# rafaelsoStanford/State_Policy_DiffusionModel

Hardware: AMD Instinct MI355X
Metric: denoise-steps/sec (B=4096, horizon=32) (higher is better)
Workload: dtype f32 (split-fp16 MFMA operands, fp32 accumulate)

## Files before the change

state_policy_diffusionmodel_amd/csrc/conv_gemm.hip:

```cpp
#include <algorithm>
#include <cstdlib>

#include "device_utils.h"

namespace spdm {

typedef float f32x16 __attribute__((ext_vector_type(16)));
typedef float f32x4 __attribute__((ext_vector_type(4)));
typedef float f32x2 __attribute__((ext_vector_type(2)));
typedef unsigned u32x2 __attribute__((ext_vector_type(2)));
typedef _Float16 f16x8 __attribute__((ext_vector_type(8)));
typedef _Float16 f16x4 __attribute__((ext_vector_type(4)));

constexpr float SPLIT_ACT_SCALE = 16.0f;
constexpr float SPLIT_DESCALE = 1.0f / 2048.0f;

typedef _Float16 f16x2 __attribute__((ext_vector_type(2)));
__device__ __forceinline__ f32x2 split_pair(float a, float b) {
    unsigned h, l;
    split_pair_f16(a * SPLIT_ACT_SCALE, b * SPLIT_ACT_SCALE, h, l);
    return f32x2{__builtin_bit_cast(float, h), __builtin_bit_cast(float, l)};
}

constexpr int CK = 32;
// ... 563 lines not shown
                v += bias4;
                if (epi == EPI_BIAS_GELU) {
                    v.x = gelu_erf(v.x); v.y = gelu_erf(v.y); v.z = gelu_erf(v.z); v.w = gelu_erf(v.w);
                }
                if (epi == EPI_BIAS_RESID)
                    v += *reinterpret_cast<const f32x4*>(a.resid + (size_t)row * a.resid_ld + n0 + c4o * 4);
                *reinterpret_cast<f32x4*>(dstp + (size_t)row * dst_ld + n0 + c4o * 4) = v;
                if (a.row_stats != nullptr) {
                    float s1 = (v.x + v.y) + (v.z + v.w);
                    float s2 = (v.x * v.x + v.y * v.y) + (v.z * v.z + v.w * v.w);
#pragma unroll
                    for (int o2 = TPR >> 1; o2 > 0; o2 >>= 1) {
                        s1 += __shfl_xor(s1, o2, 64);
                        s2 += __shfl_xor(s2, o2, 64);
                    }
                    if (c4o == 0) {
                        double* rs = a.row_stats + ((size_t)row * n_ntiles + ntile) * 2;
                        rs[0] = (double)s1;
                        rs[1] = (double)s2;
                    }
                }
            }
        }
    }
    SPDM_STAMP()
#ifdef SPDM_DIAG
    if (stamping) a.stamps[(tid >> 8) * 128 + 127] = (unsigned long long)nstamp;
#endif
#undef SPDM_STAMP
#undef SPDM_ROW
}

int spdm_tune(int idx, int dflt) {
    constexpr int NT = 26;
    static int val[NT];
    static bool have[NT], init = false;
    if (!init) {
        for (int i = 0; i < NT; ++i) {
            char name[20];
            snprintf(name, sizeof(name), "SPDM_TUNE%d", i);
            const char* e = getenv(name);
            have[i] = e != nullptr;
            val[i] = e ? atoi(e) : 0;
        }
        init = true;
    }
    return (idx >= 0 && idx < NT && have[idx]) ? val[idx] : dflt;
}

GemmGeom gemm_geometry(int M, int N, int K, int HW, int W, int taps, int split, unsigned sw, bool stats_epi) {
    GemmGeom g;
    g.skinny = 0;
    g.reg = 0;
    if (stats_epi && conv_reg_geometry(M, N, K, HW, W, taps, split, sw)) {
        g.reg = 1;
        g.m_tile = 64; g.n_tile = 64; g.n_tiles = 1; g.ksplit = 1;
        g.st_m_tile = 64; g.st_n_tiles = 1;
        g.slots = stats_slots(HW, 64, 1);
        return g;
    }
    if (stats_epi && taps != 1 && conv_skinny_geometry(M, N, K, HW, W, taps, split, sw, &g.m_tile, &g.n_tile)) {
        g.skinny = 1;
        g.ksplit = 1;
        g.n_tiles = N / g.n_tile;
        g.st_m_tile = g.m_tile;
        g.st_n_tiles = g.n_tiles;
        g.slots = stats_slots(HW, g.st_m_tile, g.st_n_tiles);
// ... 80 lines not shown
    return conv_wide_takes_upcat(b, g);
}

bool gemm_takes_two_sources(const GemmArgs& a0) {
    if (a0.skip == nullptr || !a0.split || a0.wgt_frag == nullptr || (a0.sw & SW_NO_FUSED_SRC) || a0.epi != EPI_STATS) return false;
    GemmArgs a = a0;
    const GemmGeom g = gemm_geometry(a);
    if (g.skinny || g.reg || g.m_tile == 512) return false;
    a.ksplit = g.ksplit;
    return conv_wide_supported(a, g);
}

static bool uses_w2(const GemmArgs& a, const GemmGeom& g) {
    return a.split && g.m_tile == 256 && a.taps == 9 && a.W == 2 && a.HW % 2 == 0 && !(a.sw & SW_NO_W2);
}
static bool uses_wp4(const GemmArgs& a0, const GemmGeom& g) {
    if (!(a0.split && a0.taps == 9 && a0.W == 4 && g.n_tile == 128 && (g.m_tile == 128 || g.m_tile == 256) && a0.HW % 16 == 0 &&
          a0.K % 64 == 0 && !(a0.sw & SW_NO_WP4)) || g.skinny) return false;
    GemmArgs a = a0;
    a.ksplit = g.ksplit;
    return conv_wide_supported(a, g);
}
static bool uses_wp8(const GemmArgs& a0, const GemmGeom& g) {
    if (!(a0.split && a0.taps == 9 && a0.W == 8 && g.n_tile == 128 && g.m_tile == 256 && a0.HW % 32 == 0 && a0.K % 64 == 0 &&
          !(a0.sw & SW_NO_WP8)) || g.skinny) return false;
    GemmArgs a = a0;
    a.ksplit = g.ksplit;
    return conv_wide_supported(a, g);
}
double gemm_flops(const GemmArgs& a0) {
    GemmArgs a = a0;
    const GemmGeom g = gemm_geometry(a.geom_M > 0 ? a.geom_M : a.M, a.N, a.K, a.HW, a.W, a.taps, a.split, a.sw, a.epi == EPI_STATS);
    if (a.pro == PRO_UPCAT && !g.skinny && gemm_takes_fused_source(a0)) a.pro = a.skip_stats.p != nullptr ? PRO_GN : PRO_NONE;
    const double taps = uses_w2(a, g) ? 6.0 : uses_wp4(a, g) ? 7.5 : uses_wp8(a, g) ? 8.25 : (double)a.taps;
    return 2.0 * (double)a.M * (double)a.N * (double)a.K * taps;
}

template <bool HALO, int PREC, int WM, int WN, int MT, int NT, int TPI, bool W2 = false, bool DEEP = false>
static hipError_t launch_cfg(const GemmArgs& a, const GemmGeom& g, hipStream_t s) {
    constexpr int M_T = WM * MT * 32, N_T = WN * NT * 32, NTHR = WM * WN * 64;
    constexpr int NBA = (TPI == 1 || DEEP) ? 2 : 1;
    const int halo = HALO ? a.W + 1 : 0;
    const int QA = M_T + 2 * halo;
    const int NSP = (QA + 4) & ~3;
#ifdef SPDM_WDMA
    constexpr bool WDMA = (NTHR == 512) && (PREC == PREC_SPLIT);
#else
    constexpr bool WDMA = false;
#endif
    constexpr int WROW = WDMA ? 32 : LDK;
    size_t lds = (size_t)(NBA * (QA + 1) * LDK + 2 * TPI * N_T * WROW + 2 * NSP) * sizeof(float);
    lds = std::max(lds, (size_t)(M_T * WN * 2 + M_T * N_T) * sizeof(float));
    if (lds > 160 * 1024 || g.m_tile != M_T || g.n_tile != N_T) return hipErrorInvalidValue;
    auto kern = conv_gemm_kernel<HALO, PREC, WM, WN, MT, NT, TPI, W2, DEEP>;
    if (hipError_t e = allow_full_lds(reinterpret_cast<const void*>(kern)); e != hipSuccess) return e;
    const int n_mtiles = (a.M + M_T - 1) / M_T;
    const int grid = n_mtiles * g.n_tiles * std::max(a.ksplit, 1);
    if (a.route) *a.route = GemmRoute{ROUTE_GEMM, W2 ? VAR_W2 : VAR_PLAIN, M_T, N_T};
    hipLaunchKernelGGL(kern, dim3(grid), dim3(NTHR), lds, s, a, g.slots);
    return hipGetLastError();
}

static hipError_t launch_gemm_kernel(const GemmArgs& a, const GemmGeom& g, hipStream_t s);

static int g_wide_upcat_launches = 0;
int gemm_wide_upcat_launches() { return g_wide_upcat_launches; }

// ... 80 lines not shown
```

state_policy_diffusionmodel_amd/csrc/conv_wide.hip:

```cpp
#include <algorithm>
#include <cstdlib>

#include "device_utils.h"
#include "resample.h"

namespace spdm {

typedef float f32x16 __attribute__((ext_vector_type(16)));
typedef float f32x4 __attribute__((ext_vector_type(4)));
typedef float f32x2 __attribute__((ext_vector_type(2)));
typedef _Float16 f16x8 __attribute__((ext_vector_type(8)));
typedef _Float16 f16x2 __attribute__((ext_vector_type(2)));

namespace {

constexpr float ACT_SCALE = 16.0f;
constexpr float DESCALE = 1.0f / 2048.0f;
constexpr int CK = 32;
#ifndef WIDE_LDS_PERM
#define WIDE_LDS_PERM 1
#endif
template <bool W2, bool PIPE = false, bool WP = false> struct WidePitch { static constexpr int value = (W2 || PIPE || WP || !WIDE_LDS_PERM) ? 36 : 40; };
constexpr bool wp_active(int t, int rt) { return !((t % 3 == 0 && (rt & 3) == 0) || (t % 3 == 2 && (rt & 3) == 3)); }
constexpr int wp_first(int t) { return (t % 3 == 0) ? 1 : 0; }
// ... 12 lines not shown
#ifndef WIDE_STAGE_GROUP
#define WIDE_STAGE_GROUP 1
#endif
#ifndef WIDE_DB
#define WIDE_DB 0
#endif
#ifndef WIDE_EARLY
#define WIDE_EARLY 0
#endif
#ifndef WIDE_NH
#define WIDE_NH 2
#endif

__device__ __forceinline__ f32x2 split2(float a, float b) {
    unsigned h, l;
    split_pair_f16(a * ACT_SCALE, b * ACT_SCALE, h, l);
    return f32x2{__builtin_bit_cast(float, h), __builtin_bit_cast(float, l)};
}

template <int NT, int PRO, bool W2, int RT, int WN, bool PIPE, bool TWO = false, int WP = 0, bool G2 = false, int WH = 0, bool UP = false>
#ifndef WIDE_MINB
#define WIDE_MINB 2
#endif
__global__ __launch_bounds__(256, WIDE_MINB) void conv3x3_wide_kernel(const GemmArgs a, const int epi_slots, const int NS) {
    constexpr int WM = 4 / WN;
    constexpr int CT = 2 * NT;
    constexpr int RW = RT * 16;
    constexpr int NTHR = 256;
    constexpr int RP = NTHR / 8;
    constexpr int M_T = WM * RW, N_T = WN * NT * 32;
    constexpr bool WHOLE = (WH != 0);
    constexpr bool ONE = (WH == 2);
    constexpr int APASS = WHOLE ? M_T / RP : (M_T + 18 + RP - 1) / RP;
    constexpr int FAR = (W2 || WP) ? 4 : 3;
    constexpr int FBR = (NT == 2) ? 2 : 3;
    constexpr int PH = 3 * NT;
    constexpr int BB = (APASS <= 9) ? 7 : (APASS <= 10) ? 6 : 5;
    static_assert(APASS * BB <= 64, "sample-index packing");
    static_assert(!W2 || NT == 2, "the width-2 variant exists for 128-wide tiles");
    static_assert(RT == 8 || (RT == 4 && NT == 2 && !W2), "64-row waves only in the tap-pair loop");
    static_assert(WN == 2 || (WN == 1 && RT == 4), "the 4 x 1 wave arrangement uses 64-row waves");
    static_assert(!TWO || (!PIPE && PRO != PRO_GN_GELU), "two-source input: first conv of a block, plain hand-over");
    static_assert(WP == 0 || WP == 4 || WP == 8, "row permutation for width-4 or width-8 maps");
    static_assert(!WP || (NT == 2 && WN == 2 && !W2 && !PIPE), "row permutation: 128-wide tiles");
    static_assert((16 + 4 * (WP == 8 ? 7 : 6)) % 4 == 0, "A ring phase");
    static_assert(WP != 8 || RT == 8, "width-8 maps: one 128-row block per wave");
    constexpr bool WP8 = (WP == 8);
    constexpr int NI8 = (M_T + 18 + 6) / 8 + 1;
    static_assert(!G2 || (NT == 2 && RT == 4 && !W2 && !PIPE && !WP && !WIDE_DB), "two chunks per hand-over: the plain tap loop, 64 rows per wave");
    static_assert(!WHOLE || (!G2 && !WIDE_DB && !WIDE_EARLY), "whole-sample staging: not in the hand-over experiments");
    static_assert(!UP || (TWO && WHOLE && RT == 8 && NT == 2 && WN == 2 && (W2 || WP)), "upsample in the loader: whole-sample two-source 256-row tiles");
    constexpr int UW = WP8 ? 8 : WP ? 4 : 2;
    constexpr int UPASS = M_T / 4 / RP;
    constexpr int RAWP = 36;
    extern __shared__ __attribute__((aligned(16))) float smem[];

    const int tid = threadIdx.x, lane = tid & 63;
    const int wave = __builtin_amdgcn_readfirstlane(tid >> 6);
    const int wm = wave / WN, wn = wave % WN, l16 = lane & 15, kg = lane >> 4;
    const int HW = a.HW, W = a.W, H = a.H, M = a.M, K = a.K, N = a.N;
    const int halo = WHOLE ? 0 : W + 1;
    const int QA = M_T + 2 * halo;
    const int QZ = WP8 ? 8 * NI8 + 2 : QA + 2;

    const int n_ntiles = N / N_T;
    const int nblk = gridDim.x, bid = blockIdx.x;
    const int q8 = nblk >> 3, r8 = nblk & 7, xcd = bid & 7, idx = bid >> 3;
    const int logical = (xcd < r8 ? xcd * (q8 + 1) : r8 * (q8 + 1) + (xcd - r8) * q8) + idx;
    const int ksp = a.ksplit > 1 ? a.ksplit : 1;
    const int tiles_mn = nblk / ksp;
    const int ks = logical / tiles_mn, tl = logical - ks * tiles_mn;
    const int mtile = tl / n_ntiles, ntile = tl - mtile * n_ntiles;
    const int m0 = mtile * M_T, n0 = ntile * N_T;
    const int kc0 = 2 * (int)((long long)ks * (K / (2 * CK)) / ksp), kc1 = (ksp > 1) ? 2 * (int)((long long)(ks + 1) * (K / (2 * CK)) / ksp) : K / CK;

    static_assert(!PIPE || (NT == 2 && !W2), "the pipelined hand-over exists in the tap loop of 128-wide tiles");
    constexpr int LDK = WidePitch<W2, PIPE, (WP != 0) || G2>::value;
// ... 242 lines not shown
        acc[rt_][(ct0_)] = __builtin_amdgcn_mfma_f32_16x16x32_f16(fa[fas_][0], fb[fbs_][0][0], acc[rt_][(ct0_)], 0, 0, 0);         \
        acc[rt_][(ct0_) + 1] = __builtin_amdgcn_mfma_f32_16x16x32_f16(fa[fas_][0], fb[fbs_][1][0], acc[rt_][(ct0_) + 1], 0, 0, 0); \
        acc[rt_][(ct0_)] = __builtin_amdgcn_mfma_f32_16x16x32_f16(fa[fas_][0], fb[fbs_][0][1], acc[rt_][(ct0_)], 0, 0, 0);         \
        acc[rt_][(ct0_) + 1] = __builtin_amdgcn_mfma_f32_16x16x32_f16(fa[fas_][0], fb[fbs_][1][1], acc[rt_][(ct0_) + 1], 0, 0, 0); \
        acc[rt_][(ct0_)] = __builtin_amdgcn_mfma_f32_16x16x32_f16(fa[fas_][1], fb[fbs_][0][0], acc[rt_][(ct0_)], 0, 0, 0);         \
        acc[rt_][(ct0_) + 1] = __builtin_amdgcn_mfma_f32_16x16x32_f16(fa[fas_][1], fb[fbs_][1][0], acc[rt_][(ct0_) + 1], 0, 0, 0); \
    }

    const int nrows = (kc1 - kc0) * 3;
    f16x8 fa[FAR][2], fb[FBR][2][2];
#define WIDE_SHIFT(kr_, dwi_) (WP8 ? (((dwi_) - 1) * NI8 + ((kr_) - 1)) * LDK : (((kr_) - 1) * W + ((dwi_) - 1)) * LDK)

    if constexpr (!W2 && NT == 2 && !(WP && RT == 8)) {
        f16x8 fbt[2][4][2], fat[2][2];
#define TAP_LOAD_B(slot_, chunk_, tap_)                                                              \
        if (!dbg_no_wload) {                                                                         \
            const float* p_ = wfl + (size_t)((tap_) * nchunks + (chunk_)) * wtap;                    \
            _Pragma("unroll") for (int c_ = 0; c_ < 4; ++c_) {                                      \
                fbt[slot_][c_][0] = *reinterpret_cast<const f16x8*>(p_ + c_ * 512);                  \
                fbt[slot_][c_][1] = *reinterpret_cast<const f16x8*>(p_ + c_ * 512 + 256);            \
            }                                                                                        \
        }
#define TAP_LOAD_FA(slot_, tap_, shift_, rt_)                                                        \
        {                                                                                            \
            const unsigned mb_ = (am[(rt_) / 3] >> (9 * ((rt_) % 3) + (tap_))) & 1u;                 \
            const int o_ = mb_ ? aoff0 + WIDE_ROWOFF(rt_) * LDK + (shift_) : zoff;                   \
            fat[slot_][0] = *reinterpret_cast<const f16x8*>(Abuf + o_);                              \
            fat[slot_][1] = *reinterpret_cast<const f16x8*>(Abuf + o_ + 16);                         \
        }
        const int TAPS = a.taps;
        const bool t3 = (TAPS == 3);
#define TAP_SHIFT(tap_) (t3 ? ((tap_) - 1) * W * LDK : (((tap_) / 3 - 1) * W + ((tap_) - ((tap_) / 3) * 3 - 1)) * LDK)
#define TAP_BIT(tap_) (t3 ? 3 * (tap_) + 1 : (tap_))
        if constexpr (WP) {
#define WP_SHIFT(t_) ((((t_) / 3 - 1) * W + ((t_) % 3 - 1)) * LDK)
            TAP_LOAD_B(0, kc0, 0)
            WIDE_LOAD_A(kc0)
            WIDE_STAGE_A()
            __syncthreads();
            WIDE_STAMP(2)
            int aoff_w = aoff0;
#define WP_LOAD_FA(slot_, tap_, shift_, rt_)                                                         \
            {                                                                                        \
                const unsigned mb_ = (am[(rt_) / 3] >> (9 * ((rt_) % 3) + (tap_))) & 1u;             \
                const int o_ = mb_ ? aoff_w + WIDE_ROWOFF(rt_) * LDK + (shift_) : zoff;              \
                fat[slot_][0] = *reinterpret_cast<const f16x8*>(Abuf + o_);                          \
                fat[slot_][1] = *reinterpret_cast<const f16x8*>(Abuf + o_ + 16);                     \
            }
            WP_LOAD_FA(0, 0, WP_SHIFT(0), wp_first(0))
            for (int chunk = kc0; chunk < kc1; ++chunk) {
                const int cn1 = min(chunk + 1, kc1 - 1);
                asm volatile("" : "+v"(aoff_w));
#pragma unroll
                for (int i = 0; i < (RT + 2) / 3; ++i) asm volatile("" : "+v"(am[i]));
#pragma unroll
                for (int t = 0; t < 9; ++t) {
                    if (t < 8) { TAP_LOAD_B((t + 1) & 1, chunk, t + 1) } else { TAP_LOAD_B(1, cn1, 0) }
#pragma unroll
                    for (int rt = 0; rt < RT; ++rt) {
                        {
                            if (wp_active(t, rt)) {
                                const int g = wp_order(t, rt, RT);
                                const int nx = wp_next(t, rt, RT);
                                if (nx >= 0) { WP_LOAD_FA((g + 1) & 1, t, WP_SHIFT(t), nx) }
                                else if (t < 8) { WP_LOAD_FA((g + 1) & 1, t + 1, WP_SHIFT(t + 1), wp_first(t + 1)) }
                                __builtin_amdgcn_sched_barrier(0);
                                if (!dbg_no_mfma) {
// ... 58 lines not shown
                    const int bi_ = WHOLE ? ((pass_) * RP + srow_p) >> lhw : (int)((abidx >> (BB * (pass_))) & ((1ull << BB) - 1)); \
                    const float rs_ = srstd[bi_], mu_ = smean[bi_];                                  \
                    v_.x = (v_.x - mu_) * (rs_ * g4r.x) + b4r.x;                                     \
                    v_.y = (v_.y - mu_) * (rs_ * g4r.y) + b4r.y;                                     \
                    v_.z = (v_.z - mu_) * (rs_ * g4r.z) + b4r.z;                                     \
                    v_.w = (v_.w - mu_) * (rs_ * g4r.w) + b4r.w;                                     \
                }                                                                                    \
                if (pro) {                                                                           \
                    if (pro_gelu) {                                                                  \
                        v_.x = gelu_erf(v_.x); v_.y = gelu_erf(v_.y);                                \
                        v_.z = gelu_erf(v_.z); v_.w = gelu_erf(v_.w);                                \
                    }                                                                                \
                }                                                                                    \
                if (!WHOLE && !((avalid >> (pass_)) & 1u)) v_ = f32x4{0.f, 0.f, 0.f, 0.f};              \
                const f32x2 p0_ = split2(v_.x, v_.y), p1_ = split2(v_.z, v_.w);                      \
                float* row_ = Awr + (WHOLE ? (pass_) * RP + srow_p : min((pass_) * RP + srow_p, QA + 1)) * LDK; \
                *reinterpret_cast<f32x2*>(row_ + c4 * 2) = f32x2{p0_.x, p1_.x};                      \
                *reinterpret_cast<f32x2*>(row_ + 16 + c4 * 2) = f32x2{p0_.y, p1_.y};                 \
            }
#define PIPE_SHIFT(t_) ((((t_) / 3 - 1) * W + ((t_) % 3 - 1)) * LDK)
            TAP_LOAD_B(0, kc0, 0)
            WIDE_LOAD_A(kc0)
            WIDE_STAGE_A()
            __syncthreads();
            { float* t_ = Abuf; Abuf = Awr; Awr = t_; }
            {
                const int c1 = min(kc0 + 1, kc1 - 1);
                PIPE_LOAD(0, c1, 0)
                PIPE_LOAD(1, c1, 1)
                PIPE_LOAD(2, c1, 2)
                PIPE_GB(c1)
            }
            WIDE_STAMP(2)
            PIPE_LOAD_FA(0, 0, PIPE_SHIFT(0), 0)
            for (int chunk = kc0; chunk < kc1; ++chunk) {
                const int cn1 = min(chunk + 1, kc1 - 1), cn2 = min(chunk + 2, kc1 - 1);
                PIPE_OPAQUE()
#pragma unroll
                for (int t = 0; t < 9; ++t) {
                    if (t < 8) { TAP_LOAD_B((t + 1) & 1, chunk, t + 1) } else { TAP_LOAD_B(1, cn1, 0) }
                    if (t < APASS) { PIPE_STAGE(t % 3, t) }
                    if (t + 3 < APASS) { PIPE_LOAD(t % 3, cn1, t + 3) }
                    else if (t >= 6) { PIPE_LOAD(t - 6, cn2, t - 6) }
                    if (t == 8) { PIPE_GB(cn2) }
#pragma unroll
                    for (int rt = 0; rt < RT; ++rt) {
                        if (rt + 1 < RT) { PIPE_LOAD_FA((rt + 1) & 1, t, PIPE_SHIFT(t), rt + 1) }
                        else if (t < 8) { PIPE_LOAD_FA(0, t + 1, PIPE_SHIFT(t + 1), 0) }
                        __builtin_amdgcn_sched_barrier(0);
#pragma unroll
                        for (int c = 0; c < 4; ++c)
                            acc[rt][c] = __builtin_amdgcn_mfma_f32_16x16x32_f16(fat[rt & 1][0], fbt[t & 1][c][0], acc[rt][c], 0, 0, 0);
#pragma unroll
                        for (int c = 0; c < 4; ++c)
                            acc[rt][c] = __builtin_amdgcn_mfma_f32_16x16x32_f16(fat[rt & 1][0], fbt[t & 1][c][1], acc[rt][c], 0, 0, 0);
#pragma unroll
                        for (int c = 0; c < 4; ++c)
                            acc[rt][c] = __builtin_amdgcn_mfma_f32_16x16x32_f16(fat[rt & 1][1], fbt[t & 1][c][0], acc[rt][c], 0, 0, 0);
                        __builtin_amdgcn_sched_barrier(0);
                    }
                }
                __syncthreads();
                { float* t_ = Abuf; Abuf = Awr; Awr = t_; }
#pragma unroll
                for (int c = 0; c < 4; ++c) { fbt[0][c][0] = fbt[1][c][0]; fbt[0][c][1] = fbt[1][c][1]; }
                PIPE_LOAD_FA(0, 0, PIPE_SHIFT(0), 0)
            }
#undef PIPE_OPAQUE
#undef PIPE_LOAD_FA
#undef PIPE_LOAD
#undef PIPE_GB
#undef PIPE_STAGE
#undef PIPE_SHIFT
        } else if constexpr (G2) {
        const int ntaps = (kc1 - kc0) * TAPS;
        f32x4 areg2[APASS];
        f32x4 g4r2 = {1.f, 1.f, 1.f, 1.f}, b4r2 = {0.f, 0.f, 0.f, 0.f};
        bool ident2 = false;
        const float* Acur = Abuf;
#define G2_LOAD_FA(slot_, tap_, shift_, rt_)                                                         \
        {                                                                                            \
            const unsigned mb_ = (am[(rt_) / 3] >> (9 * ((rt_) % 3) + (tap_))) & 1u;                 \
            const int o_ = mb_ ? aoff0 + WIDE_ROWOFF(rt_) * LDK + (shift_) : zoff;                   \
            fat[slot_][0] = *reinterpret_cast<const f16x8*>(Acur + o_);                              \
            fat[slot_][1] = *reinterpret_cast<const f16x8*>(Acur + o_ + 16);                         \
        }
        TAP_LOAD_B(0, kc0, 0)
        WIDE_LOAD_A_(kc0, areg, g4r, b4r, ident)
        WIDE_LOAD_A_(min(kc0 + 1, kc1 - 1), areg2, g4r2, b4r2, ident2)
        WIDE_STAGE_A_(areg, g4r, b4r, ident, Abuf)
        WIDE_STAGE_A_(areg2, g4r2, b4r2, ident2, Abuf + QZ * LDK)
        __syncthreads();
        WIDE_STAMP(2)
        G2_LOAD_FA(0, TAP_BIT(0), TAP_SHIFT(0), 0)
        int chunk = kc0, tap = 0;
        for (int tt = 0; tt < ntaps; tt += 2) {
#pragma unroll
            for (int half = 0; half < 2; ++half) {
                int ntap = tap + 1, nchunk = chunk;
// ... 66 lines not shown
                    __builtin_amdgcn_sched_barrier(0);
                    if (!dbg_no_mfma) {
#pragma unroll
                        for (int c = 0; c < 4; ++c)
                            acc[rt][c] = __builtin_amdgcn_mfma_f32_16x16x32_f16(fat[rt & 1][0], fbt[half][c][0], acc[rt][c], 0, 0, 0);
#pragma unroll
                        for (int c = 0; c < 4; ++c)
                            acc[rt][c] = __builtin_amdgcn_mfma_f32_16x16x32_f16(fat[rt & 1][0], fbt[half][c][1], acc[rt][c], 0, 0, 0);
#pragma unroll
                        for (int c = 0; c < 4; ++c)
                            acc[rt][c] = __builtin_amdgcn_mfma_f32_16x16x32_f16(fat[rt & 1][1], fbt[half][c][0], acc[rt][c], 0, 0, 0);
                    }
                    __builtin_amdgcn_sched_barrier(0);
                }
                if (next_A && !dbg_no_aload) {
                    if (!(DB && WIDE_EARLY)) { WIDE_LOAD_A(nchunk) }
                    if (!DB) __syncthreads();
                    WIDE_STAGE_A()
                    __syncthreads();
                    if (DB) { float* t_ = Abuf; Abuf = Awr; Awr = t_; }
                    TAP_LOAD_FA(0, TAP_BIT(0), TAP_SHIFT(0), 0)
                } else if (next_A) {
                    TAP_LOAD_FA(0, TAP_BIT(0), TAP_SHIFT(0), 0)
                }
                tap = ntap;
                chunk = nchunk;
            }
        }
        }
#undef TAP_LOAD_B
#undef TAP_LOAD_FA
#undef TAP_SHIFT
#undef TAP_BIT
    } else if constexpr (WP) {
#define WP_PLUS(i_) (WP8 ? (i_) : (i_) + (i_) / 3)
#define WP_MINUS(i_) (WP8 ? (i_) + 1 : (i_) + (i_) / 3 + 1)
        constexpr int WS = WP8 ? 7 : 6;
        constexpr int Q1 = 16 + 2 * WS, Q2 = 16 + 4 * WS;
        WIDE_LOAD_B(0, kc0, 1, 0)
        WIDE_LOAD_A(kc0)
        WIDE_STAGE_A()
        __syncthreads();
        WIDE_STAMP(2)
        WIDE_LOAD_FA(0, 1, WIDE_SHIFT(0, 1), 0)
        WIDE_LOAD_FA(1, 1, WIDE_SHIFT(0, 1), 1)
        int chunk = kc0, kr = 0;
        for (int r = 0; r < nrows; ++r) {
            int nkr = kr + 1, nchunk = chunk;
            if (nkr == 3) { nkr = 0; nchunk = chunk + 1; }
            const bool have_next = (r + 1 < nrows);
            const bool next_A = have_next && (nkr == 0);
            const int bkr = have_next ? nkr : kr, bchunk = have_next ? nchunk : chunk;
#pragma unroll
            for (int cp = 0; cp < 2; ++cp) {
                if (cp == 0) { WIDE_LOAD_B(1, chunk, kr * 3 + 1, 1) } else { WIDE_LOAD_B(0, chunk, kr * 3 + 2, 0) }
#pragma unroll
                for (int rt = 0; rt < RT; ++rt) {
                    const int q = cp * 8 + rt;
                    if (q + 2 < 16) { WIDE_LOAD_FA((q + 2) % FAR, kr * 3 + 1, WIDE_SHIFT(kr, 1), (q + 2) % 8) }
                    else { WIDE_LOAD_FA((q + 2) % FAR, kr * 3 + 2, WIDE_SHIFT(kr, 2), WP_PLUS(q + 2 - 16)) }
                    __builtin_amdgcn_sched_barrier(0);
                    WIDE_STEP(q % FAR, cp, rt, cp * 2)
                    __builtin_amdgcn_sched_barrier(0);
                }
            }
#pragma unroll
// ... 336 lines not shown
            a.skip_ld < a.K - a.up_C || a.src_ld < a.up_C) return false;
    }
    if (a.ksplit > 1 && a.K % 64 != 0) return false;
    if ((g.m_tile + 2 * (a.W + 1) - 1) / a.HW + 2 > 128) return false;
    if (g.m_tile == 128)
        return g.n_tile == 128 && (a.taps == 9 || (a.taps == 3 && a.W == 1)) && a.K % 64 == 0 && !(a.sw & SW_NO_WIDE128);
    if (g.m_tile != 256) return false;
    if (a.taps == 3) return false;
    if (a.taps != 9 || !(g.n_tile == 128 || g.n_tile == 64)) return false;
    if (wide_w2(a)) return g.n_tile == 128 && (a.HW & 7) == 0;
    if (g.n_tile == 128 && a.K % 64 != 0) return false;
    return true;
}

static GemmArgs upcat_as_two(const GemmArgs& a0) {
    GemmArgs a = a0;
    a.pro = a0.skip_stats.p != nullptr ? PRO_GN : PRO_NONE;
    return a;
}
bool conv_wide_takes_upcat(const GemmArgs& a, const GemmGeom& g) {
    if (a.pro != PRO_UPCAT || a.M <= 0 || a.skip == nullptr || a.src == nullptr || g.skinny || g.reg || g.ksplit > 1 || a.ksplit > 1) return false;
    if (g.m_tile != 256 || g.n_tile != 128 || a.taps != 9 || (a.H & 1) || a.HW != a.H * a.W || a.HW < 16 || (a.HW & (a.HW - 1)) != 0) return false;
    if ((a.sw & (SW_NO_WHOLE_TILES | SW_NO_FUSED_SRC)) || 256 % a.HW != 0 || a.M % 256 != 0 || a.K % 64 != 0) return false;
    const int level = a.W == 8 ? 0 : a.W == 4 ? 1 : a.W == 2 ? 2 : -1;
    if (level < 0 || !((spdm_tune(22, 7) >> level) & 1)) return false;
    if ((a.W == 8 && ((a.sw & SW_NO_WP8) || a.HW % 32 != 0)) || (a.W == 4 && ((a.sw & SW_NO_WP4) || a.HW % 16 != 0)) ||
        (a.W == 2 && (a.sw & SW_NO_W2))) return false;
    if (a.pro_stats.p != nullptr && (a.pro_gamma == nullptr || a.pro_beta == nullptr || a.pro_stats.HW * 4 != a.HW)) return false;
    if (a.skip_stats.p != nullptr && (a.skip_gamma == nullptr || a.skip_beta == nullptr || a.skip_stats.HW != a.HW)) return false;
    if (a.src_ld % 4 != 0 || a.dst_ld % 4 != 0 || a.N % 128 != 0) return false;
    return conv_wide_supported(upcat_as_two(a), g);
}

hipError_t launch_conv_wide(const GemmArgs& a0, const GemmGeom& g, hipStream_t s) {
    if (a0.pro == PRO_UPCAT) {
        if (!conv_wide_takes_upcat(a0, g)) return hipErrorInvalidValue;
        const GemmArgs a = upcat_as_two(a0);
        if (a.W == 8) {
            if (a.pro == PRO_NONE) return launch_wide_sel<3, 2, PRO_NONE, false, 8, 2, false, true, 8, true>(a, g, s);
            return launch_wide_sel<3, 2, PRO_GN, false, 8, 2, false, true, 8, true>(a, g, s);
        }
        if (a.W == 4) {
            if (a.pro == PRO_NONE) return launch_wide_sel<1, 2, PRO_NONE, false, 8, 2, false, true, 4, true>(a, g, s);
            return launch_wide_sel<1, 2, PRO_GN, false, 8, 2, false, true, 4, true>(a, g, s);
        }
        if (a.pro == PRO_NONE) return launch_wide_sel<1, 2, PRO_NONE, true, 8, 2, false, true, 0, true>(a, g, s);
        return launch_wide_sel<1, 2, PRO_GN, true, 8, 2, false, true, 0, true>(a, g, s);
    }
    const GemmArgs& a = a0;
    if (!conv_wide_supported(a, g)) return hipErrorInvalidValue;
    const bool pipe = a.taps == 9 && a.K >= 256 && !(a.sw & SW_NO_WIDE_PIPE);
    if (a.W == 4 && a.taps == 9 && g.n_tile == 128 && a.HW % 16 == 0 && a.K % 64 == 0 && !(a.sw & SW_NO_WP4)) {
        const bool two = a.skip != nullptr;
        if (g.m_tile == 128) {
            if (two) {
                if (a.pro == PRO_NONE) return launch_wide_sel<1, 2, PRO_NONE, false, 4, 2, false, true, 4>(a, g, s);
                return launch_wide_sel<1, 2, PRO_GN, false, 4, 2, false, true, 4>(a, g, s);
            }
            if (a.pro == PRO_NONE) return launch_wide_sel<1, 2, PRO_NONE, false, 4, 2, false, false, 4>(a, g, s);
            if (a.pro == PRO_GN) return launch_wide_sel<1, 2, PRO_GN, false, 4, 2, false, false, 4>(a, g, s);
            return launch_wide_sel<1, 2, PRO_GN_GELU, false, 4, 2, false, false, 4>(a, g, s);
        }
        if (two) {
            if (a.pro == PRO_NONE) return launch_wide_sel<1, 2, PRO_NONE, false, 8, 2, false, true, 4>(a, g, s);
            return launch_wide_sel<1, 2, PRO_GN, false, 8, 2, false, true, 4>(a, g, s);
        }
// ... 14 lines not shown
        if (g.m_tile == 128) {
            if (a.pro == PRO_NONE) return launch_wide_sel<1, 2, PRO_NONE, false, 4, 2, false, true>(a, g, s);
            return launch_wide_sel<1, 2, PRO_GN, false, 4, 2, false, true>(a, g, s);
        }
        if (wide_w2(a)) {
            if (a.pro == PRO_NONE) return launch_wide_sel<1, 2, PRO_NONE, true, 8, 2, false, true>(a, g, s);
            return launch_wide_sel<1, 2, PRO_GN, true, 8, 2, false, true>(a, g, s);
        }
        if (a.pro == PRO_NONE) return launch_wide_cfg<2, PRO_NONE, false, 8, 2, false, true>(a, g, s);
        return launch_wide_cfg<2, PRO_GN, false, 8, 2, false, true>(a, g, s);
    }
    const bool g2 = a.K >= 64 && (a.sw & SW_G2);
    if (g.m_tile == 128) {
        if (g2) {
            if (a.pro == PRO_NONE) return launch_wide_cfg<2, PRO_NONE, false, 4, 2, false, false, false, true>(a, g, s);
            if (a.pro == PRO_GN) return launch_wide_cfg<2, PRO_GN, false, 4, 2, false, false, false, true>(a, g, s);
            return launch_wide_cfg<2, PRO_GN_GELU, false, 4, 2, false, false, false, true>(a, g, s);
        }
        if (a.pro == PRO_NONE) return launch_wide_sel<1, 2, PRO_NONE, false, 4>(a, g, s);
        if (a.pro == PRO_GN) return launch_wide_sel<1, 2, PRO_GN, false, 4>(a, g, s);
        return launch_wide_sel<1, 2, PRO_GN_GELU, false, 4>(a, g, s);
    }
    if (wide_w2(a)) {
        if (a.pro == PRO_NONE) return launch_wide_sel<1, 2, PRO_NONE, true>(a, g, s);
        if (a.pro == PRO_GN) return launch_wide_sel<1, 2, PRO_GN, true>(a, g, s);
        return launch_wide_sel<1, 2, PRO_GN_GELU, true>(a, g, s);
    }
    if (g.n_tile == 128) {
        if (a.pro == PRO_NONE) return launch_wide_cfg<2, PRO_NONE>(a, g, s);
        if (a.pro == PRO_GN) return launch_wide_cfg<2, PRO_GN>(a, g, s);
        return launch_wide_cfg<2, PRO_GN_GELU>(a, g, s);
    }
    if (a.K % 64 == 0 && !(a.sw & SW_WIDE_N64_2X2)) {
        if (pipe) {
            if (a.pro == PRO_NONE) return launch_wide_sel<3, 2, PRO_NONE, false, 4, 1, true>(a, g, s);
            if (a.pro == PRO_GN) return launch_wide_sel<3, 2, PRO_GN, false, 4, 1, true>(a, g, s);
            return launch_wide_sel<3, 2, PRO_GN_GELU, false, 4, 1, true>(a, g, s);
        }
        if (g2) {
            if (a.pro == PRO_NONE) return launch_wide_cfg<2, PRO_NONE, false, 4, 1, false, false, false, true>(a, g, s);
            if (a.pro == PRO_GN) return launch_wide_cfg<2, PRO_GN, false, 4, 1, false, false, false, true>(a, g, s);
            return launch_wide_cfg<2, PRO_GN_GELU, false, 4, 1, false, false, false, true>(a, g, s);
        }
        if (a.pro == PRO_NONE) return launch_wide_sel<3, 2, PRO_NONE, false, 4, 1>(a, g, s);
        if (a.pro == PRO_GN) return launch_wide_sel<3, 2, PRO_GN, false, 4, 1>(a, g, s);
        return launch_wide_sel<3, 2, PRO_GN_GELU, false, 4, 1>(a, g, s);
    }
    if (a.pro == PRO_NONE) return launch_wide_cfg<1, PRO_NONE>(a, g, s);
    if (a.pro == PRO_GN) return launch_wide_cfg<1, PRO_GN>(a, g, s);
    return launch_wide_cfg<1, PRO_GN_GELU>(a, g, s);
}

}
```

state_policy_diffusionmodel_amd/csrc/kernels.h:

```cpp
#pragma once
#include <hip/hip_runtime.h>
#include <stdint.h>
#include <mutex>
#include <set>
#include <utility>
#include <vector>

namespace spdm {

inline hipError_t allow_full_lds(const void* kern) {
    static std::mutex mu;
    static std::set<std::pair<int, const void*>> done;
    int dev = 0;
    hipError_t e = hipGetDevice(&dev);
    if (e != hipSuccess) return e;
    std::lock_guard<std::mutex> lk(mu);
    if (done.count({dev, kern})) return hipSuccess;
    e = hipFuncSetAttribute(kern, hipFuncAttributeMaxDynamicSharedMemorySize, (int)(160 * 1024));
    if (e == hipSuccess) done.insert({dev, kern});
    return e;
}

struct StatsRef {
    const double* p;
// ... 65 lines not shown
};
enum { DBG_NO_MFMA = 1, DBG_NO_WLOAD = 2, DBG_NO_GELU = 4, DBG_NO_STORE = 8, DBG_NO_ALOAD = 16, DBG_PP = 64, DBG_STAMP = 128 };

struct GemmGeom {
    int m_tile, n_tile, n_tiles;
    int slots;
    int ksplit;
    int skinny;
    int reg;
    int st_m_tile, st_n_tiles;
};
GemmGeom gemm_geometry(int M, int N, int K, int HW, int W, int taps, int split, unsigned sw, bool stats_epi = false);
GemmGeom gemm_geometry(const GemmArgs& a);
constexpr size_t SPLITK_WORKSPACE_BYTES = (size_t)48 << 20;
__host__ __device__ inline int combine_rows(int HW, int N) {
    int r = HW;
    while ((r & 1) == 0 && (long long)r * N > 2048) r >>= 1;
    return r;
}
bool conv_skinny_geometry(int M, int N, int K, int HW, int W, int taps, int split, unsigned sw, int* m_tile, int* n_tile);
hipError_t launch_conv_skinny(const GemmArgs& a, const GemmGeom& g, hipStream_t s);
bool conv_reg_geometry(int M, int N, int K, int HW, int W, int taps, int split, unsigned sw);
hipError_t launch_conv_reg64(const GemmArgs& a, const GemmGeom& g, hipStream_t s);
inline bool pooled_stats_serial(const StatsRef& st) {
    return st.m_tile > 0 && st.HW % st.m_tile == 0 && (st.HW / st.m_tile) * st.n_tiles <= 8;
}
hipError_t launch_splitk_combine(const float* partial, int ksplit, float* dst, int M, int N, int HW, double* stats,
                                 hipStream_t s);
hipError_t launch_gemm(const GemmArgs& a, hipStream_t s);
bool gemm_takes_fused_source(const GemmArgs& a);
bool gemm_takes_two_sources(const GemmArgs& a);
double gemm_flops(const GemmArgs& a);
bool conv_wide_supported(const GemmArgs& a, const GemmGeom& g);
bool conv_wide_takes_upcat(const GemmArgs& a, const GemmGeom& g);
int gemm_wide_upcat_launches();
hipError_t launch_conv_wide(const GemmArgs& a, const GemmGeom& g, hipStream_t s);

constexpr int CHAIN_MAX_LAYERS = 8;
struct ChainLayer {
    const float* wfrag;
    const float* gamma;  const float* beta;
    int K, N, gelu;
};
struct ChainArgs {
    const float* src;  int src_ld;
    float* dst;        int dst_ld;
    double* stats;     int slots;
    int M, HW;
    int n_layers;
    int debug;
    ChainLayer layer[CHAIN_MAX_LAYERS];
};
constexpr int CHAIN_M_TILE = 64;
bool conv_chain_geometry(int M, int HW, int W, int taps, int split, int n_layers, const int* chan);
int conv_chain_blocks(int M);
double conv_chain_flops(const ChainArgs& a);
hipError_t launch_conv_chain(const ChainArgs& a, hipStream_t s);

int conv_in_parts(int Hp, int Wp, int B);
hipError_t launch_conv_in(const float* x, const float* w , float* dst, double* stats,
                          int B, int H0, int D, int Hp, int Wp, int lh, int lw, int* step_dev, int* t_dev,
                          const int* timesteps_dev, int n_steps, int adv, hipStream_t s, int B_geom = 0);

struct AffineSrc {
    const float* x; int C;
    StatsRef st; const float* gamma; const float* beta;
// ... 429 lines not shown
```

Before: 549,000.

## Extend zero-padding tap skipping to 64-wide conv tiles for width-4/8 maps

Extends the row-permutation scheme, which skips 3x3 conv taps that only read zero padding on width-4 and width-8 feature maps, to 64-column output tiles. It adds a new NT==1 2x2-wave schedule for width 8 and permuted-row support for the pipelined and non-pipelined 4x1 arrangement at width 4. It also updates the FLOP accounting. The path is gated by a new tune knob and by shape conditions (GN prologue, no skip input, whole tiles, at least 2048 samples). The goal is to drop the padding-tap MFMA work on the small-spatial U-Net layers, at the cost of more template variants and more complex scheduling.

```diff
diff --git a/state_policy_diffusionmodel_amd/csrc/conv_gemm.hip b/state_policy_diffusionmodel_amd/csrc/conv_gemm.hip
--- a/state_policy_diffusionmodel_amd/csrc/conv_gemm.hip
+++ b/state_policy_diffusionmodel_amd/csrc/conv_gemm.hip
@@ -619,7 +619,7 @@
 }
 
 int spdm_tune(int idx, int dflt) {
-    constexpr int NT = 26;
+    constexpr int NT = 27;
     static int val[NT];
     static bool have[NT], init = false;
     if (!init) {
@@ -766,7 +766,10 @@
     GemmArgs a = a0;
     const GemmGeom g = gemm_geometry(a.geom_M > 0 ? a.geom_M : a.M, a.N, a.K, a.HW, a.W, a.taps, a.split, a.sw, a.epi == EPI_STATS);
     if (a.pro == PRO_UPCAT && !g.skinny && gemm_takes_fused_source(a0)) a.pro = a.skip_stats.p != nullptr ? PRO_GN : PRO_NONE;
-    const double taps = uses_w2(a, g) ? 6.0 : uses_wp4(a, g) ? 7.5 : uses_wp8(a, g) ? 8.25 : (double)a.taps;
+    GemmArgs aw = a;
+    aw.ksplit = g.ksplit;
+    const int skip64 = (!g.skinny && !g.reg && conv_wide_supported(aw, g)) ? conv_wide_skip64(aw, g) : 0;
+    const double taps = uses_w2(a, g) ? 6.0 : (uses_wp4(a, g) || skip64 == 4) ? 7.5 : (uses_wp8(a, g) || skip64 == 8) ? 8.25 : (double)a.taps;
     return 2.0 * (double)a.M * (double)a.N * (double)a.K * taps;
 }
 
diff --git a/state_policy_diffusionmodel_amd/csrc/conv_wide.hip b/state_policy_diffusionmodel_amd/csrc/conv_wide.hip
--- a/state_policy_diffusionmodel_amd/csrc/conv_wide.hip
+++ b/state_policy_diffusionmodel_amd/csrc/conv_wide.hip
@@ -68,7 +68,7 @@
     constexpr bool WHOLE = (WH != 0);
     constexpr bool ONE = (WH == 2);
     constexpr int APASS = WHOLE ? M_T / RP : (M_T + 18 + RP - 1) / RP;
-    constexpr int FAR = (W2 || WP) ? 4 : 3;
+    constexpr int FAR = (W2 || (WP && NT == 2)) ? 4 : 3;
     constexpr int FBR = (NT == 2) ? 2 : 3;
     constexpr int PH = 3 * NT;
     constexpr int BB = (APASS <= 9) ? 7 : (APASS <= 10) ? 6 : 5;
@@ -78,7 +78,9 @@
     static_assert(WN == 2 || (WN == 1 && RT == 4), "the 4 x 1 wave arrangement uses 64-row waves");
     static_assert(!TWO || (!PIPE && PRO != PRO_GN_GELU), "two-source input: first conv of a block, plain hand-over");
     static_assert(WP == 0 || WP == 4 || WP == 8, "row permutation for width-4 or width-8 maps");
-    static_assert(!WP || (NT == 2 && WN == 2 && !W2 && !PIPE), "row permutation: 128-wide tiles");
+    static_assert(!WP || (!W2 && ((NT == 2 && (WN == 2 ? !PIPE : (WP == 4 && RT == 4))) || (NT == 1 && WN == 2 && RT == 8 && !PIPE))),
+                  "row permutation: 128-wide tiles; 64-wide: width 4 on the 4 x 1 arrangement (one 64-row block per wave, either hand-over), "
+                  "or 2 x 2 waves of 128 rows x 32 columns");
     static_assert((16 + 4 * (WP == 8 ? 7 : 6)) % 4 == 0, "A ring phase");
     static_assert(WP != 8 || RT == 8, "width-8 maps: one 128-row block per wave");
     constexpr bool WP8 = (WP == 8);
@@ -387,7 +389,7 @@
         const bool t3 = (TAPS == 3);
 #define TAP_SHIFT(tap_) (t3 ? ((tap_) - 1) * W * LDK : (((tap_) / 3 - 1) * W + ((tap_) - ((tap_) / 3) * 3 - 1)) * LDK)
 #define TAP_BIT(tap_) (t3 ? 3 * (tap_) + 1 : (tap_))
-        if constexpr (WP) {
+        if constexpr (WP && !PIPE) {
 #define WP_SHIFT(t_) ((((t_) / 3 - 1) * W + ((t_) % 3 - 1)) * LDK)
             TAP_LOAD_B(0, kc0, 0)
             WIDE_LOAD_A(kc0)
@@ -512,7 +514,7 @@
                 PIPE_GB(c1)
             }
             WIDE_STAMP(2)
-            PIPE_LOAD_FA(0, 0, PIPE_SHIFT(0), 0)
+            PIPE_LOAD_FA(0, 0, PIPE_SHIFT(0), WP ? wp_first(0) : 0)
             for (int chunk = kc0; chunk < kc1; ++chunk) {
                 const int cn1 = min(chunk + 1, kc1 - 1), cn2 = min(chunk + 2, kc1 - 1);
                 PIPE_OPAQUE()
@@ -525,26 +527,30 @@
                     if (t == 8) { PIPE_GB(cn2) }
 #pragma unroll
                     for (int rt = 0; rt < RT; ++rt) {
-                        if (rt + 1 < RT) { PIPE_LOAD_FA((rt + 1) & 1, t, PIPE_SHIFT(t), rt + 1) }
-                        else if (t < 8) { PIPE_LOAD_FA(0, t + 1, PIPE_SHIFT(t + 1), 0) }
-                        __builtin_amdgcn_sched_barrier(0);
-#pragma unroll
-                        for (int c = 0; c < 4; ++c)
-                            acc[rt][c] = __builtin_amdgcn_mfma_f32_16x16x32_f16(fat[rt & 1][0], fbt[t & 1][c][0], acc[rt][c], 0, 0, 0);
-#pragma unroll
-                        for (int c = 0; c < 4; ++c)
-                            acc[rt][c] = __builtin_amdgcn_mfma_f32_16x16x32_f16(fat[rt & 1][0], fbt[t & 1][c][1], acc[rt][c], 0, 0, 0);
-#pragma unroll
-                        for (int c = 0; c < 4; ++c)
-                            acc[rt][c] = __builtin_amdgcn_mfma_f32_16x16x32_f16(fat[rt & 1][1], fbt[t & 1][c][0], acc[rt][c], 0, 0, 0);
-                        __builtin_amdgcn_sched_barrier(0);
+                        if (!WP || wp_active(t, rt)) {
+                            const int g = WP ? wp_order(t, rt, RT) : rt;
+                            const int nx = WP ? wp_next(t, rt, RT) : (rt + 1 < RT ? rt + 1 : -1);
+                            if (nx >= 0) { PIPE_LOAD_FA((g + 1) & 1, t, PIPE_SHIFT(t), nx) }
+                            else if (t < 8) { PIPE_LOAD_FA((g + 1) & 1, t + 1, PIPE_SHIFT(t + 1), WP ? wp_first(t + 1) : 0) }
+                            __builtin_amdgcn_sched_barrier(0);
+#pragma unroll
+                            for (int c = 0; c < 4; ++c)
+                                acc[rt][c] = __builtin_amdgcn_mfma_f32_16x16x32_f16(fat[g & 1][0], fbt[t & 1][c][0], acc[rt][c], 0, 0, 0);
+#pragma unroll
+                            for (int c = 0; c < 4; ++c)
+                                acc[rt][c] = __builtin_amdgcn_mfma_f32_16x16x32_f16(fat[g & 1][0], fbt[t & 1][c][1], acc[rt][c], 0, 0, 0);
+#pragma unroll
+                            for (int c = 0; c < 4; ++c)
+                                acc[rt][c] = __builtin_amdgcn_mfma_f32_16x16x32_f16(fat[g & 1][1], fbt[t & 1][c][0], acc[rt][c], 0, 0, 0);
+                            __builtin_amdgcn_sched_barrier(0);
+                        }
                     }
                 }
                 __syncthreads();
                 { float* t_ = Abuf; Abuf = Awr; Awr = t_; }
 #pragma unroll
                 for (int c = 0; c < 4; ++c) { fbt[0][c][0] = fbt[1][c][0]; fbt[0][c][1] = fbt[1][c][1]; }
-                PIPE_LOAD_FA(0, 0, PIPE_SHIFT(0), 0)
+                PIPE_LOAD_FA(0, 0, PIPE_SHIFT(0), WP ? wp_first(0) : 0)
             }
 #undef PIPE_OPAQUE
 #undef PIPE_LOAD_FA
@@ -677,6 +683,67 @@
 #undef TAP_LOAD_FA
 #undef TAP_SHIFT
 #undef TAP_BIT
+    } else if constexpr (WP && NT == 1) {
+#define WP_PLUS(i_) (WP8 ? (i_) : (i_) + (i_) / 3)
+#define WP_MINUS(i_) (WP8 ? (i_) + 1 : (i_) + (i_) / 3 + 1)
+        constexpr int WS = WP8 ? 7 : 6;
+        constexpr int RS = 8 + 2 * WS;
+        static_assert((3 * RS) % FAR == 0 && 9 % FBR == 0, "A / B ring phase from chunk to chunk");
+        WIDE_LOAD_B(0, kc0, 0, 0)
+        WIDE_LOAD_A(kc0)
+        WIDE_STAGE_A()
+        __syncthreads();
+        WIDE_STAMP(2)
+        WIDE_LOAD_FA(0, 0, WIDE_SHIFT(0, 0), WP_MINUS(0))
+        WIDE_LOAD_FA(1, 0, WIDE_SHIFT(0, 0), WP_MINUS(1))
+        for (int chunk = kc0; chunk < kc1; ++chunk) {
+            const bool have_next = (chunk + 1 < kc1);
+            const int bchunk = have_next ? chunk + 1 : chunk;
+#pragma unroll
+            for (int kr = 0; kr < 3; ++kr) {
+                const int s0 = kr * RS;
+                WIDE_LOAD_B((3 * kr + 1) % FBR, chunk, kr * 3 + 1, 0)
+#pragma unroll
+                for (int i = 0; i < WS; ++i) {
+                    const int s = s0 + i;
+                    if (i + 2 < WS) { WIDE_LOAD_FA((s + 2) % FAR, kr * 3, WIDE_SHIFT(kr, 0), WP_MINUS(i + 2)) }
+                    else { WIDE_LOAD_FA((s + 2) % FAR, kr * 3 + 1, WIDE_SHIFT(kr, 1), i + 2 - WS) }
+                    __builtin_amdgcn_sched_barrier(0);
+                    WIDE_STEP(s % FAR, (3 * kr) % FBR, WP_MINUS(i), 0)
+                    __builtin_amdgcn_sched_barrier(0);
+                }
+                WIDE_LOAD_B((3 * kr + 2) % FBR, chunk, kr * 3 + 2, 0)
+#pragma unroll
+                for (int rt = 0; rt < RT; ++rt) {
+                    const int s = s0 + WS + rt;
+                    if (rt + 2 < 8) { WIDE_LOAD_FA((s + 2) % FAR, kr * 3 + 1, WIDE_SHIFT(kr, 1), rt + 2) }
+                    else { WIDE_LOAD_FA((s + 2) % FAR, kr * 3 + 2, WIDE_SHIFT(kr, 2), WP_PLUS(rt + 2 - 8)) }
+                    __builtin_amdgcn_sched_barrier(0);
+                    WIDE_STEP(s % FAR, (3 * kr + 1) % FBR, rt, 0)
+                    __builtin_amdgcn_sched_barrier(0);
+                }
+                if (kr < 2) { WIDE_LOAD_B(0, chunk, (kr + 1) * 3, 0) } else { WIDE_LOAD_B(0, bchunk, 0, 0) }
+#pragma unroll
+                for (int i = 0; i < WS; ++i) {
+                    const int s = s0 + WS + 8 + i;
+                    if (i + 2 < WS) { WIDE_LOAD_FA((s + 2) % FAR, kr * 3 + 2, WIDE_SHIFT(kr, 2), WP_PLUS(i + 2)) }
+                    else if (kr < 2) { WIDE_LOAD_FA((s + 2) % FAR, (kr + 1) * 3, WIDE_SHIFT(kr + 1, 0), WP_MINUS(i + 2 - WS)) }
+                    __builtin_amdgcn_sched_barrier(0);
+                    WIDE_STEP(s % FAR, (3 * kr + 2) % FBR, WP_PLUS(i), 0)
+                    __builtin_amdgcn_sched_barrier(0);
+                }
+            }
+            if (have_next) {
+                WIDE_LOAD_A(chunk + 1)
+                __syncthreads();
+                WIDE_STAGE_A()
+                __syncthreads();
+                WIDE_LOAD_FA(0, 0, WIDE_SHIFT(0, 0), WP_MINUS(0))
+                WIDE_LOAD_FA(1, 0, WIDE_SHIFT(0, 0), WP_MINUS(1))
+            }
+        }
+#undef WP_PLUS
+#undef WP_MINUS
     } else if constexpr (WP) {
 #define WP_PLUS(i_) (WP8 ? (i_) : (i_) + (i_) / 3)
 #define WP_MINUS(i_) (WP8 ? (i_) + 1 : (i_) + (i_) / 3 + 1)
@@ -1079,6 +1146,17 @@
     return conv_wide_supported(upcat_as_two(a), g);
 }
 
+constexpr int WIDE64_SKIP_DEFAULT = 3;
+constexpr int WIDE64_SKIP_MIN_SAMPLES = 2048;
+int conv_wide_skip64(const GemmArgs& a, const GemmGeom& g) {
+    const int tune = spdm_tune(26, WIDE64_SKIP_DEFAULT);
+    if (g.n_tile != 64 || g.m_tile != 256 || a.taps != 9 || !(a.W == 4 || a.W == 8) || a.HW % (4 * a.W) != 0 || a.K % 64 != 0) return 0;
+    if (!((tune >> (a.W == 8 ? 0 : 1)) & 1) || (a.sw & (a.W == 8 ? SW_NO_WP8 : SW_NO_WP4)) || (a.sw & SW_WIDE_N64_2X2)) return 0;
+    if (a.skip != nullptr || a.pro != PRO_GN || a.ksplit > 1) return 0;
+    if (!(tune & 8) && ((a.sw & SW_NO_WHOLE_TILES) || a.HW != 4 * a.W * a.W || a.M % 256 != 0 || a.M / a.HW < WIDE64_SKIP_MIN_SAMPLES)) return 0;
+    return a.W;
+}
+
 hipError_t launch_conv_wide(const GemmArgs& a0, const GemmGeom& g, hipStream_t s) {
     if (a0.pro == PRO_UPCAT) {
         if (!conv_wide_takes_upcat(a0, g)) return hipErrorInvalidValue;
@@ -1159,6 +1237,12 @@
         return launch_wide_cfg<2, PRO_GN_GELU>(a, g, s);
     }
     if (a.K % 64 == 0 && !(a.sw & SW_WIDE_N64_2X2)) {
+        if (const int wskip = conv_wide_skip64(a, g); wskip == 4) {
+            if (pipe && (spdm_tune(26, WIDE64_SKIP_DEFAULT) & 4)) return launch_wide_sel<1, 2, PRO_GN, false, 4, 1, true, false, 4>(a, g, s);
+            return launch_wide_sel<1, 2, PRO_GN, false, 4, 1, false, false, 4>(a, g, s);
+        } else if (wskip == 8) {
+            return launch_wide_sel<3, 1, PRO_GN, false, 8, 2, false, false, 8>(a, g, s);
+        }
         if (pipe) {
             if (a.pro == PRO_NONE) return launch_wide_sel<3, 2, PRO_NONE, false, 4, 1, true>(a, g, s);
             if (a.pro == PRO_GN) return launch_wide_sel<3, 2, PRO_GN, false, 4, 1, true>(a, g, s);
diff --git a/state_policy_diffusionmodel_amd/csrc/kernels.h b/state_policy_diffusionmodel_amd/csrc/kernels.h
--- a/state_policy_diffusionmodel_amd/csrc/kernels.h
+++ b/state_policy_diffusionmodel_amd/csrc/kernels.h
@@ -121,6 +121,7 @@
 bool gemm_takes_two_sources(const GemmArgs& a);
 double gemm_flops(const GemmArgs& a);
 bool conv_wide_supported(const GemmArgs& a, const GemmGeom& g);
+int conv_wide_skip64(const GemmArgs& a, const GemmGeom& g);
 bool conv_wide_takes_upcat(const GemmArgs& a, const GemmGeom& g);
 int gemm_wide_upcat_launches();
 hipError_t launch_conv_wide(const GemmArgs& a, const GemmGeom& g, hipStream_t s);
```

After: 553,100, median of 6. About the same (+0.7%).
